# tuffy/libdvd-audio

Hardware: AMD Instinct MI355X
Metric: decoded PCM Msamples/s (bit-exact) on 6ch/96k/24b MLP (higher is better)
Workload: dtype int32 (int64 accumulate)

## Files before the change

### libdvd-audio_amd/csrc/mlp_ctx.h

```cpp
#pragma once
#include <vector>

#include "hip_ws.h"
#include "mlp_decode.h"
#include "mlp_conceal.h"
#include "mlp_index.h"

using namespace mlp;

constexpr uint32_t EV_RING = 256;
constexpr uint32_t SEQ_ROUND = 1024;

struct DecodeSettings {
    uint32_t lanes_per_seg = 0;
    uint32_t pcm_layout = DVDA_PCM_PLANAR;
    uint32_t chain_form = 0;
    const int32_t *d_init_fir = nullptr;
};

struct ConcealInfo {
    uint32_t valid, status;
    uint64_t rows, frames;
};

struct ConcealState {
    bool on = false;
    dvda_mlp_hip_ctx *child = nullptr;
    DevBuf<ConcealPlan> d_plan;
    DevBuf<uint8_t> d_bytes;
    DevBuf<uint64_t> d_tab;
    DevBuf<int32_t> d_scr[CONCEAL_ROUNDS];
    DevBuf<ConcealOp> d_ops;
    DevBuf<int32_t> d_fir;
    DevBuf<int32_t> d_edge_fir;
    bool ran = false;
    std::vector<StreamRec> h_streams;
    std::vector<dvda_mlp_conceal_edges> edges;
    std::vector<std::vector<dvda_mlp_conceal_span>> spans;
    std::vector<ConcealInfo> info;

    ~ConcealState() { dvda_mlp_hip_destroy(child); }
};

struct PresentState {
    uint32_t mode = DVDA_PRESENT_FULL;
    dvda_mlp_hip_ctx *child = nullptr;
    DevBuf<uint8_t> d_bytes;
    uint64_t bound = 0;
    DevBuf<uint32_t> d_info;
    DevBuf<uint32_t> d_size;
    DevBuf<uint32_t> d_sbase;
    DevBuf<uint32_t> d_len;
    DevBuf<uint32_t> d_base;
    DevBuf<uint64_t> d_off64, d_len64;
    Event ev[2];
    bool ev_set = false;
    bool map_valid = false;
    uint32_t h_nseg = 0;
    std::vector<SegRec> h_seg;
    std::vector<uint32_t> h_sbase, h_base, h_info;
    std::vector<StreamRec> h_streams;

    ~PresentState() { dvda_mlp_hip_destroy(child); }
};

struct dvda_mlp_hip_ctx {
    int device;
    uint32_t coop_min_seg;
    uint32_t max_streams, max_segments;
    DevBuf<uint8_t> d_masks;
    DevBuf<uint16_t> d_parts;
    DevBuf<uint32_t> d_tile_count;
    DevBuf<uint32_t> d_tile_base;
    DevBuf<uint64_t> d_cand_off;
    DevBuf<SegRec> d_seg;
    DevBuf<uint32_t> d_seg_frames;
    DevBuf<uint32_t> d_seg_fbase;
    DevBuf<uint32_t> d_seg_status;
    DevBuf<uint32_t> d_seg_rows;
    DevBuf<StreamRec> d_streams;
    uint32_t *d_n_cand;
    DevBuf<uint32_t> d_scan_tmp;
    DevBuf<int32_t> d_iir;
    DevBuf<uint32_t> d_mat;
    DevBuf<unsigned long long> d_dbg;
    DevBuf<int32_t> d_fir;
    DevBuf<uint32_t> d_seg_meta;
    DevBuf<uint32_t> d_yield;
    DevBuf<uint32_t> d_seg_check;
    DevBuf<uint32_t> d_cls;
    DevBuf<uint32_t> d_shape_key;
    DevBuf<uint64_t> d_soff, d_slen;
    DevBuf<uint32_t> d_rank;
    DevBuf<uint32_t> d_sorted_cnt;
    DevBuf<uint32_t> d_sorted_base;
    DevBuf<uint32_t> d_lane_seg;
    DevBuf<DecodeSummary> d_summary;
    DecodeSummary *h_summary;
    Stream st_aux;
    Event ev_fork, ev_join;
    DevBuf<uint32_t> d_seq_list;
    DevBuf<uint4> d_plan;
    DevBuf<uint4> d_scan4_tmp;
    DevBuf<uint32_t> d_def_list;
    DevBuf<uint32_t> d_head_list;
    DevBuf<uint32_t> d_chain_order;
    DevBuf<uint32_t> d_chain_hist;
    DevBuf<int32_t> d_fb;
    uint32_t rsv_segs;
    DevBuf<int32_t> d_res;
    DevBuf<uint32_t> d_brec;
    DevBuf<uint32_t> d_frec;
    uint32_t iir_lanes;
    DevBuf<dvda_pcm_crc_desc> d_rep_desc;
    DevBuf<uint64_t> d_rep_out;
    DevBuf<uint32_t> d_rep_work;
    DecodeSettings set;
    const uint8_t *d_bytes;
    uint64_t total_bytes;
    const uint64_t *d_stream_off;
    const uint64_t *d_stream_len;
    uint32_t n_streams;
    uint64_t tiles;
    bool indexed;
    bool small_input;
    bool decoded;
    GraphExec idx_graph;
    const void *idx_key[4];
    uint64_t idx_key_bytes;
    uint32_t idx_key_streams;
    int idx_graph_state;
    Event ev[2 * EV_RING];
    Event ev_end[EV_RING];
    uint64_t ev_count;
    ConcealState cc;
    PresentState pp;

    uint32_t fb_slots() const { return (uint32_t)(d_fb.cap / FB_WORDS); }
    ~dvda_mlp_hip_ctx() { (void)hipHostFree(h_summary); }
};

static WsCaps ws_caps(const dvda_mlp_hip_ctx *c)
{
    WsCaps w;
    w.res = c->d_res.cap;
    w.brec = c->d_brec.cap;
    w.frec = c->d_frec.cap;
    w.fb = c->d_fb.cap;
    w.max_seg = c->max_segments;
    w.max_streams = c->max_streams;
    w.lanes = c->iir_lanes;
    w.pad = 0;
    return w;
}

static inline dvda_mlp_hip_ctx *pp_inner(const dvda_mlp_hip_ctx *c)
{
    return c && c->pp.mode == DVDA_PRESENT_SUBSTREAM0 ? c->pp.child : nullptr;
}

// ... 24 lines not shown
```

### libdvd-audio_amd/csrc/mlp_hip.hip

```cpp
#include <hip/hip_runtime.h>
#include <math.h>
#include <stdint.h>
#include <stdio.h>
#include <stdlib.h>
#include <string.h>
#include <new>
#include <vector>

#include "../../include/dvda_mlp_hip.h"
#include "mlp_step.h"
#include "mlp_decode.h"
#include "mlp_chain.h"
#include "mlp_chain_small.h"
#include "mlp_check.h"
#include "mlp_coop.h"
#include "mlp_index.h"
#include "mlp_conceal.h"
#include "mlp_present.h"
#include "pcm_unswizzle.h"
#include "wav_pack.h"
#include "pcm_digest.h"
#include "pcm_levels.h"

#include "mlp_ctx.h"
#include "mlp_conceal_run.h"
#include "mlp_present_run.h"
#include "mlp_stepper.h"
#include "mlp_tiers.h"
#include "pcm_report_run.h"

extern "C" int dvda_mlp_hip_bounds_violations(unsigned long long *out4)
{
    if (!out4)
        return DVDA_HIP_EINVAL;
    out4[0] = out4[1] = out4[2] = out4[3] = 0;
#if defined(DVDA_BOUNDS)
    HIP_TRY(hipDeviceSynchronize());
    HIP_TRY(hipMemcpyFromSymbol(out4, HIP_SYMBOL(mlp::g_bounds), 4 * sizeof(unsigned long long)));
    return 1;
#else
    return DVDA_HIP_OK;
#endif
}

extern "C" const char *dvda_mlp_hip_version(void) { return "dvda-mlp-hip 0.1 (gfx950)"; }

extern "C" int dvda_mlp_hip_create(dvda_mlp_hip_ctx **out, int device, uint32_t max_streams,
                                   uint32_t max_segments)
{
    if (!out || max_streams == 0 || max_segments == 0)
        return DVDA_HIP_EINVAL;
    int ndev = 0;
    if (hipGetDeviceCount(&ndev) != hipSuccess || ndev <= 0 || device < 0 || device >= ndev) {
        fprintf(stderr, "dvda_mlp_hip: no usable HIP device (count=%d, requested=%d)\n", ndev, device);
        return DVDA_HIP_ENODEV;
    }
    HIP_TRY(hipSetDevice(device));
    dvda_mlp_hip_ctx *c = new (std::nothrow) dvda_mlp_hip_ctx();
    if (!c)
        return DVDA_HIP_ENOMEM;
    c->device = device;
    {
        int cus = 0;
        if (hipDeviceGetAttribute(&cus, hipDeviceAttributeMultiprocessorCount, device) != hipSuccess || cus <= 0)
            cus = 256;
        c->coop_min_seg = (uint32_t)cus * 4u * 64u * 7u / 4u;
        if (const char *e = getenv("DVDA_COOP_MIN_SEG"))
            c->coop_min_seg = (uint32_t)strtoul(e, nullptr, 10);
    }
    c->max_streams = max_streams;
    c->max_segments = max_segments;
    c->idx_graph_state = getenv("DVDA_INDEX_GRAPH") && atoi(getenv("DVDA_INDEX_GRAPH")) == 0 ? -1 : 0;
    const size_t ns = (size_t)max_segments, nt = (size_t)max_streams;
    c->iir_lanes = (uint32_t)(((2 * ns + DEC_THREADS - 1) / DEC_THREADS) * DEC_THREADS);
    const size_t nl = c->iir_lanes;
    hipError_t e = hipSuccess;
    auto alloc = [&](auto &buf, size_t n) {
        if (e == hipSuccess)
            e = buf.alloc(n);
    };
    alloc(c->d_cand_off, ns);
    alloc(c->d_seg, ns + 4);
    alloc(c->d_seg_frames, ns + 1);
    alloc(c->d_seg_fbase, ns + 5);
    alloc(c->d_seg_status, ns + 4);
    alloc(c->d_seg_rows, ns);
    alloc(c->d_streams, nt);
    alloc(c->d_iir, nl * MAXCH * 16);
    alloc(c->d_mat, nl * MAXMAT * 5);
    alloc(c->d_dbg, 32);
    alloc(c->d_fir, nl * 6 * 8);
    alloc(c->d_seg_meta, nl + 4);
    alloc(c->d_yield, ns);
    alloc(c->d_seg_check, 2 * ns);
    alloc(c->d_cls, 4);
    alloc(c->d_shape_key, nt);
    alloc(c->d_soff, nt);
    alloc(c->d_slen, nt);
    alloc(c->d_rank, nt);
    alloc(c->d_sorted_cnt, nt + 1);
    alloc(c->d_sorted_base, nt + 1);
    alloc(c->d_lane_seg, ns);
    alloc(c->d_summary, 1 + SUMMARY_PARTS);
    alloc(c->d_seq_list, nt);
    alloc(c->d_plan, ns + 5);
    alloc(c->d_scan4_tmp, ns / 1024 + 4);
    alloc(c->d_def_list, ns);
    alloc(c->d_head_list, ns);
    alloc(c->d_chain_order, ns);
    alloc(c->d_chain_hist, 2 * CHAIN_BUCKETS);
    if (e == hipSuccess)
        e = hipHostMalloc((void **)&c->h_summary, sizeof(DecodeSummary), hipHostMallocDefault);
    if (e == hipSuccess)
        e = hipStreamCreateWithFlags(c->st_aux.put(), hipStreamNonBlocking);
    if (e == hipSuccess)
        e = hipEventCreateWithFlags(c->ev_fork.put(), hipEventDisableTiming);
    if (e == hipSuccess)
        e = hipEventCreateWithFlags(c->ev_join.put(), hipEventDisableTiming);
    if (e == hipSuccess)
        e = hipMemset(c->d_dbg, 0, 32 * sizeof(unsigned long long));
    if (e == hipSuccess)
        e = hipMemset(c->d_seg_meta, 0, nl * sizeof(uint32_t));
    for (uint32_t i = 0; e == hipSuccess && i < 2 * EV_RING; i++)
        e = hipEventCreate(c->ev[i].put());
    for (uint32_t i = 0; e == hipSuccess && i < EV_RING; i++)
        e = hipEventCreate(c->ev_end[i].put());
    if (e != hipSuccess) {
        fprintf(stderr, "dvda_mlp_hip: workspace allocation failed: %s\n", hipGetErrorString(e));
        delete c;
        return DVDA_HIP_ENOMEM;
    }
    *out = c;
    return DVDA_HIP_OK;
}

extern "C" void dvda_mlp_hip_destroy(dvda_mlp_hip_ctx *c)
{
    if (!c)
        return;
    (void)hipSetDevice(c->device);
#if defined(DVDA_BOUNDS)
    if (getenv("DVDA_BOUNDS_REPORT")) {
        unsigned long long v[4] = {0, 0, 0, 0};
        (void)dvda_mlp_hip_bounds_violations(v);
        fprintf(stderr, "dvda_mlp_hip: bounds violations: %llu", v[0]);
        if (v[0])
            fprintf(stderr, " (first: tag %llu index %llu capacity %llu)", v[1], v[2], v[3]);
        fprintf(stderr, "\n");
    }
#endif
    delete c;
}

static int ensure_byte_ws(dvda_mlp_hip_ctx *c, uint64_t total_bytes)
{
    const uint64_t chunks = (total_bytes + 15) / 16 + 4;
    const uint64_t tiles = (chunks + IDX_TILE_CHUNKS - 1) / IDX_TILE_CHUNKS;
    auto grow_pair = [](auto &a, uint64_t na, auto &b, uint64_t nb) {
        if (na <= a.cap)
            return DVDA_HIP_OK;
        a.release();
        b.release();
        if (a.alloc(na) == hipSuccess && b.alloc(nb) == hipSuccess)
            return DVDA_HIP_OK;
        a.release();
        return DVDA_HIP_ENOMEM;
    };
    int rc = grow_pair(c->d_masks, chunks, c->d_parts, chunks + 72);
    if (rc)
        return rc;
    uint64_t most = tiles > c->max_segments ? tiles : c->max_segments;
    if (c->max_streams > most)
        most = c->max_streams;
    if ((rc = c->d_scan_tmp.grow_exact((most + 1023) / 1024 + 2)) != 0)
        return rc;
    return grow_pair(c->d_tile_count, tiles + 1, c->d_tile_base, tiles + 1);
}

__global__ void k_init_streams(StreamRec *s, uint32_t n, uint32_t *seg_status, uint32_t *seg_rows, uint32_t *yield_req,
                               uint32_t *seg_meta, uint32_t n_seg, uint32_t *cls, uint32_t *summary_words)
{
    const uint32_t i = blockIdx.x * blockDim.x + threadIdx.x;
    if (i < 4)
        cls[i] = 0;
    if (i < (1 + SUMMARY_PARTS) * sizeof(DecodeSummary) / sizeof(uint32_t))
        summary_words[i] = 0;
    if (i < n_seg) {
        seg_status[i] = 0;
        seg_rows[i] = 0;
        yield_req[i] = 0;
        seg_meta[2 * (size_t)i] = seg_meta[2 * (size_t)i + 1] = 0;
    }
    if (i < n) {
        StreamRec r;
        r.first_seg = 0xFFFFFFFFu;
        r.n_seg = 0;
        r.sync = 0;
        r.status = 0;
        r.frames = 0;
        r.consumed = 0;
        r.rows = 0;
        s[i] = r;
    }
}

__global__ void k_reset_segments(uint32_t *seg_status, uint32_t *seg_rows, uint32_t *yield_req, uint32_t *seg_meta,
                                 uint32_t n_seg)
{
    const uint32_t i = blockIdx.x * blockDim.x + threadIdx.x;
    if (i < n_seg) {
        seg_status[i] = 0;
        seg_rows[i] = 0;
        yield_req[i] = 0;
        seg_meta[2 * (size_t)i] = seg_meta[2 * (size_t)i + 1] = 0;
    }
}

__device__ __forceinline__ void check_ranges_block(const uint64_t *__restrict__ off, const uint64_t *__restrict__ len,
                                                   uint32_t n, uint64_t total_bytes, uint64_t *__restrict__ soff,
                                                   uint64_t *__restrict__ slen, StreamRec *__restrict__ streams,
                                                   unsigned long long *s_max)
{
    const uint32_t per = (n + 1023u) / 1024u;
    const uint32_t lo = threadIdx.x * per, hi = lo + per < n ? lo + per : n;
    auto end_of = [&](uint32_t i) {
        const uint64_t o = off[i], l = len[i];
        return (o <= total_bytes && l <= total_bytes - o && (o & 15u) == 0) ? o + l : 0;
    };
    unsigned long long m = 0;
    for (uint32_t i = lo; i < hi; i++) {
        const unsigned long long e = end_of(i);
        m = e > m ? e : m;
    }
    s_max[threadIdx.x] = m;
    __syncthreads();
    for (uint32_t d = 1; d < 1024u; d <<= 1) {
        const unsigned long long v = threadIdx.x >= d ? s_max[threadIdx.x - d] : 0ull;
        __syncthreads();
        if (v > s_max[threadIdx.x])
            s_max[threadIdx.x] = v;
        __syncthreads();
    }
    unsigned long long run = threadIdx.x ? s_max[threadIdx.x - 1] : 0ull;
    for (uint32_t i = lo; i < hi; i++) {
        const uint64_t o = off[i], l = len[i];
        const bool ok = (o & 15u) == 0 && o <= total_bytes && l <= total_bytes - o && o >= run;
        const uint64_t so = ok ? o : run;
        soff[i] = so < total_bytes ? so : total_bytes;
        slen[i] = ok ? l : 0;
        if (!ok)
            streams[i].status = ST_ENVELOPE | (1u << 16);
        const unsigned long long e = end_of(i);
        run = e > run ? e : run;
    }
}

__global__ __launch_bounds__(1024) void k_check_ranges(const uint64_t *__restrict__ off, const uint64_t *__restrict__ len,
                                                       uint32_t n, uint64_t total_bytes, uint64_t *__restrict__ soff,
                                                       uint64_t *__restrict__ slen, StreamRec *__restrict__ streams)
{
    __shared__ unsigned long long s_max[1024];
    check_ranges_block(off, len, n, total_bytes, soff, slen, streams, s_max);
}

constexpr uint64_t SMALL_INPUT_BYTES = 4096u * 1024u;

static void enqueue_index(dvda_mlp_hip_ctx *c, hipStream_t st, const uint8_t *d_bytes, uint64_t total_bytes,
                          const uint64_t *d_stream_off, const uint64_t *d_stream_len, uint32_t n_streams)
{
    const uint64_t tiles = c->tiles;
    const uint32_t ms = c->max_segments;
    {
        uint32_t n_init = n_streams > ms ? n_streams : ms;
        if (n_init < 1024)
            n_init = 1024;
        hipLaunchKernelGGL(k_init_streams, dim3((n_init + 255) / 256), dim3(256), 0, st, c->d_streams,
                           n_streams, c->d_seg_status, c->d_seg_rows, c->d_yield, c->d_seg_meta, ms, c->d_cls,
                           reinterpret_cast<uint32_t *>(c->d_summary.p));
        hipLaunchKernelGGL(k_check_ranges, dim3(1), dim3(1024), 0, st, d_stream_off, d_stream_len, n_streams, total_bytes,
                           c->d_soff, c->d_slen, c->d_streams);
        d_stream_off = c->d_soff;
        d_stream_len = c->d_slen;
    }
    hipLaunchKernelGGL(k_sync_mask, dim3((unsigned)tiles), dim3(IDX_THREADS), 0, st, d_bytes,
                       total_bytes, c->d_masks, c->d_tile_count, c->d_parts);
    enqueue_exscan(st, c->d_tile_count, c->d_tile_base, c->d_scan_tmp, (uint32_t)tiles, nullptr, (uint32_t)tiles);
    hipLaunchKernelGGL(k_sync_scatter, dim3((unsigned)tiles), dim3(IDX_THREADS), 0, st, c->d_masks,
                       total_bytes, c->d_tile_base, c->d_cand_off, ms);
    hipLaunchKernelGGL(k_chase, dim3((ms + 255) / 256), dim3(256), 0, st, d_bytes, d_stream_off,
                       d_stream_len, n_streams, c->d_cand_off, c->d_n_cand, ms, c->d_seg,
                       c->d_seg_frames, c->d_streams, c->d_cls);
    hipLaunchKernelGGL(k_mark_dead, dim3((ms + 255) / 256), dim3(256), 0, st, d_stream_off, d_stream_len,
                       c->d_n_cand, ms, c->d_seg, c->d_seg_frames, c->d_streams);
    enqueue_exscan(st, c->d_seg_frames, c->d_seg_fbase, c->d_scan_tmp, 0u, c->d_n_cand, ms);
    const bool pack = !(total_bytes <= SMALL_INPUT_BYTES);
    hipLaunchKernelGGL(k_link, dim3((ms + 255) / 256), dim3(256), 0, st, d_stream_off, d_stream_len,
                       c->d_n_cand, ms, c->d_seg, c->d_seg_fbase, c->d_streams, n_streams, c->d_shape_key,
                       c->d_cls + (pack ? 2 : 3));
    hipStream_t sp = st;
    bool forked = false;
    if (pack && st != nullptr && c->st_aux && hipEventRecord(c->ev_fork, st) == hipSuccess &&
        hipStreamWaitEvent(c->st_aux, c->ev_fork, 0) == hipSuccess) {
        sp = c->st_aux;
        forked = true;
    }
    if (pack) {
    hipLaunchKernelGGL(k_stream_rank, dim3((n_streams + 255) / 256), dim3(256), 0, sp, c->d_shape_key, c->d_streams,
                       n_streams, c->d_rank, c->d_sorted_cnt, c->d_cls + 2);
    enqueue_exscan(sp, c->d_sorted_cnt, c->d_sorted_base, c->d_scan_tmp, n_streams, nullptr, n_streams);
    (void)hipMemsetAsync(c->d_lane_seg, 0xFF, (size_t)ms * sizeof(uint32_t), sp);
    hipLaunchKernelGGL(k_lane_perm, dim3((ms + 255) / 256), dim3(256), 0, sp, c->d_seg, c->d_streams, c->d_n_cand, ms,
                       c->d_rank, c->d_sorted_base, c->d_cls + 2, c->d_lane_seg);
    }
    hipLaunchKernelGGL(k_au_check, dim3((unsigned)(((uint64_t)ms * CHK_GROUP + CHK_THREADS - 1) / CHK_THREADS)),
                       dim3(CHK_THREADS), 0, st, d_bytes, c->d_parts, c->d_seg, c->d_n_cand, ms, c->d_streams, c->d_seg_check);
    if (forked) {
        (void)hipEventRecord(c->ev_join, sp);
        (void)hipStreamWaitEvent(st, c->ev_join, 0);
    }
}

static int index_source(dvda_mlp_hip_ctx *c, const uint8_t *d_bytes, uint64_t total_bytes,
                        const uint64_t *d_stream_off, const uint64_t *d_stream_len, uint32_t n_streams, void *stream_)
{
    if (!c || !d_bytes || !d_stream_off || !d_stream_len || n_streams == 0 || total_bytes == 0)
        return DVDA_HIP_EINVAL;
    if (n_streams > c->max_streams)
        return DVDA_HIP_ECAPACITY;
    if (((uintptr_t)d_bytes & 15) != 0)
        return DVDA_HIP_EINVAL;
    hipStream_t st = (hipStream_t)stream_;
    HIP_TRY(hipSetDevice(c->device));
    c->cc.spans.clear();
    c->cc.info.clear();
    int rc = ensure_byte_ws(c, total_bytes);
    if (rc)
        return rc;
    c->d_bytes = d_bytes;
    c->total_bytes = total_bytes;
    c->d_stream_off = d_stream_off;
    c->d_stream_len = d_stream_len;
    c->n_streams = n_streams;
    const uint64_t chunks = (total_bytes + 15) / 16;
    const uint64_t tiles = (chunks + IDX_TILE_CHUNKS - 1) / IDX_TILE_CHUNKS;
    c->tiles = tiles;
    c->d_n_cand = c->d_tile_base + tiles;

    c->small_input = total_bytes <= SMALL_INPUT_BYTES;
    const bool same = c->idx_graph_state > 0 && c->idx_key[0] == d_bytes && c->idx_key[1] == d_stream_off &&
                      c->idx_key[2] == d_stream_len && c->idx_key[3] == (const void *)st &&
                      c->idx_key_bytes == total_bytes && c->idx_key_streams == n_streams;
    if (c->idx_graph_state == 2 && same) {
        if (hipGraphLaunch(c->idx_graph, st) == hipSuccess) {
            c->indexed = true;
            c->decoded = false;
            return DVDA_HIP_OK;
        }
        (void)hipGetLastError();
        c->idx_graph_state = -1;
    } else if (c->idx_graph_state == 1 && same && st != nullptr) {
        hipGraph_t g = nullptr;
        bool ok = hipStreamBeginCapture(st, hipStreamCaptureModeThreadLocal) == hipSuccess;
        if (ok) {
            enqueue_index(c, st, d_bytes, total_bytes, d_stream_off, d_stream_len, n_streams);
            ok = hipStreamEndCapture(st, &g) == hipSuccess && g != nullptr;
        }
        if (ok) {
            ok = hipGraphInstantiate(c->idx_graph.put(), g, nullptr, nullptr, 0) == hipSuccess;
        }
        if (g)
            (void)hipGraphDestroy(g);
        if (ok && hipGraphLaunch(c->idx_graph, st) == hipSuccess) {
            c->idx_graph_state = 2;
            c->indexed = true;
            c->decoded = false;
            return DVDA_HIP_OK;
        }
        (void)hipGetLastError();
        c->idx_graph_state = -1;
    } else if (c->idx_graph_state >= 0) {
        c->idx_key[0] = d_bytes;
// ... 608 lines not shown
```

### libdvd-audio_amd/csrc/mlp_index.h

```cpp
#pragma once
#include <hip/hip_runtime.h>
#include <stdint.h>
#include "mlp_tables.h"

namespace mlp {

struct SegRec {
    uint64_t off;
    uint64_t end;
    uint32_t stream;
    uint32_t nframes;
    uint32_t flags;
    uint32_t sync;
    uint32_t ndrop;
    uint32_t prev;
};
constexpr uint32_t SYNC_PARAMS = 0x00FFFFFFu;
constexpr uint32_t MAX_DROP = 64;

struct StreamRec {
    uint32_t first_seg;
    uint32_t n_seg;
    uint32_t sync;
    uint32_t status;
    uint64_t frames;
    uint64_t consumed;
    uint64_t rows;
};

constexpr int IDX_THREADS = 256;
constexpr int IDX_CHUNKS_PER_THREAD = 16;
constexpr int IDX_TILE_CHUNKS = IDX_THREADS * IDX_CHUNKS_PER_THREAD;

__device__ __forceinline__ uint32_t ld_u8(const uint8_t *p, uint64_t i) { return p[i]; }

__device__ __forceinline__ bool sync_frame_at(const uint8_t *b, uint64_t p, uint64_t limit)
{
    if (p + 32 > limit)
        return false;
    const uint32_t size = 2u * (((ld_u8(b, p) & 0x0Fu) << 8) | ld_u8(b, p + 1));
    if (size < 32)
        return false;
    if (ld_u8(b, p + 4) != 0xF8 || ld_u8(b, p + 5) != 0x72 || ld_u8(b, p + 6) != 0x6F ||
        ld_u8(b, p + 7) != 0xBB)
        return false;
    const uint32_t count = ld_u8(b, p + 20) >> 4;
    return count == 1 || count == 2;
}

__device__ __forceinline__ uint64_t ld_hdr8(const uint8_t *b, uint64_t p)
{
    const uint16_t *h = reinterpret_cast<const uint16_t *>(b + p);
    return (uint64_t)h[0] | ((uint64_t)h[1] << 16) | ((uint64_t)h[2] << 32) | ((uint64_t)h[3] << 48);
}

__device__ __forceinline__ bool sync_frame_hdr(const uint8_t *b, uint64_t p, uint64_t limit, uint64_t hdr)
{
    if (p + 32 > limit)
        return false;
    const uint32_t size = 2u * ((((uint32_t)hdr & 0x0Fu) << 8) | (((uint32_t)hdr >> 8) & 0xFFu));
    if (size < 32 || (uint32_t)(hdr >> 32) != 0xBB6F72F8u)
        return false;
    const uint32_t count = ld_u8(b, p + 20) >> 4;
    return count == 1 || count == 2;
}

__device__ __forceinline__ uint32_t packed_sync_at(const uint8_t *b, uint64_t p)
{
    return (ld_u8(b, p + 8) >> 4) | ((ld_u8(b, p + 8) & 0xFu) << 4) | ((ld_u8(b, p + 9) >> 4) << 8) |
           ((ld_u8(b, p + 9) & 0xFu) << 12) | ((ld_u8(b, p + 11) & 0x1Fu) << 16) | ((ld_u8(b, p + 20) >> 4) << 24);
}

__device__ const CheckTables d_chk = make_check();

__device__ __forceinline__ uint32_t mask_chunk(const uint8_t *__restrict__ bytes, uint64_t total_bytes, uint64_t chunk,
                                               const uint8_t *s_slice, uint32_t &part)
{
    const uint4 *q = reinterpret_cast<const uint4 *>(bytes) + chunk;
    const uint4 a = q[0], c = q[1];
    uint32_t w[8] = {a.x, a.y, a.z, a.w, c.x, c.y, c.z, c.w};
    uint32_t m = 0;
    uint32_t any = 0;
#pragma unroll
    for (int k = 1; k <= 4; k++) {
        const uint32_t y = w[k] ^ 0x72F872F8u;
        any |= (y - 0x00010001u) & ~y & 0x80008000u;
    }
    if (__builtin_expect(any != 0, 0)) {
#pragma unroll
        for (int j = 0; j < 8; j++) {
            const int h = j + 2;
            const uint32_t lo = (h & 1) ? (w[h >> 1] >> 16) : (w[h >> 1] & 0xFFFFu);
            const uint32_t hi = ((h + 1) & 1) ? (w[(h + 1) >> 1] >> 16) : (w[(h + 1) >> 1] & 0xFFFFu);
            if (lo == 0x72F8u && hi == 0xBB6Fu) {
                if (sync_frame_at(bytes, chunk * 16 + 2 * j, total_bytes))
                    m |= 1u << j;
            }
        }
    }
    uint32_t c0 = 0;
#pragma unroll
    for (int k = 0; k < 4; k++)
        c0 ^= s_slice[(15 - 4 * k) * 256 + (w[k] & 0xFFu)] ^ s_slice[(14 - 4 * k) * 256 + ((w[k] >> 8) & 0xFFu)] ^
              s_slice[(13 - 4 * k) * 256 + ((w[k] >> 16) & 0xFFu)] ^ s_slice[(12 - 4 * k) * 256 + (w[k] >> 24)];
    uint32_t px = w[0] ^ w[1] ^ w[2] ^ w[3];
    px ^= px >> 16;
    px = (px ^ (px >> 8)) & 0xFFu;
    part = c0 | (px << 8);
    return m;
}

__global__ __launch_bounds__(IDX_THREADS) void k_sync_mask(const uint8_t *__restrict__ bytes,
                                                           uint64_t total_bytes,
                                                           uint8_t *__restrict__ masks,
                                                           uint32_t *__restrict__ tile_count,
// ... 23 lines not shown
        s_cnt[threadIdx.x >> 6] = cnt;
    __syncthreads();
    if (threadIdx.x == 0) {
        uint32_t t = 0;
        for (int i = 0; i < IDX_THREADS / 64; i++)
            t += s_cnt[i];
        tile_count[blockIdx.x] = t;
    }
}

__global__ __launch_bounds__(1024) void k_exscan_u32(const uint32_t *__restrict__ in,
                                                     uint32_t *__restrict__ out, uint32_t n_host,
                                                     const uint32_t *__restrict__ n_ptr,
                                                     uint32_t n_cap)
{
    __shared__ uint32_t s_part[1024];
    uint32_t n = n_ptr ? *n_ptr : n_host;
    if (n > n_cap)
        n = n_cap;
    const uint32_t per = (n + 1023) / 1024;
    const uint32_t lo = threadIdx.x * per;
    const uint32_t hi = lo + per < n ? lo + per : n;
    uint32_t sum = 0;
    for (uint32_t i = lo; i < hi; i++)
        sum += in[i];
    s_part[threadIdx.x] = sum;
    __syncthreads();
    for (int o = 1; o < 1024; o <<= 1) {
        uint32_t v = threadIdx.x >= (uint32_t)o ? s_part[threadIdx.x - o] : 0;
        __syncthreads();
        s_part[threadIdx.x] += v;
        __syncthreads();
    }
    uint32_t run = threadIdx.x ? s_part[threadIdx.x - 1] : 0;
    for (uint32_t i = lo; i < hi; i++) {
        const uint32_t v = in[i];
        out[i] = run;
        run += v;
    }
    if (threadIdx.x == 1023)
        out[n] = s_part[1023];
}

__global__ __launch_bounds__(1024) void k_scan_blocks(const uint32_t *__restrict__ in,
                                                      uint32_t *__restrict__ out,
                                                      uint32_t *__restrict__ block_sum, uint32_t n_host,
                                                      const uint32_t *__restrict__ n_ptr, uint32_t n_cap)
{
    __shared__ uint32_t s_v[1024];
    uint32_t n = n_ptr ? *n_ptr : n_host;
    if (n > n_cap)
        n = n_cap;
    const uint32_t i = blockIdx.x * 1024 + threadIdx.x;
    const uint32_t v = i < n ? in[i] : 0;
    s_v[threadIdx.x] = v;
    __syncthreads();
    for (int o = 1; o < 1024; o <<= 1) {
        const uint32_t t = threadIdx.x >= (uint32_t)o ? s_v[threadIdx.x - o] : 0;
        __syncthreads();
        s_v[threadIdx.x] += t;
        __syncthreads();
    }
    if (i < n)
        out[i] = s_v[threadIdx.x] - v;
    if (threadIdx.x == 1023)
        block_sum[blockIdx.x] = s_v[1023];
}

__global__ __launch_bounds__(1024) void k_scan_add(uint32_t *__restrict__ out,
                                                   const uint32_t *__restrict__ block_base,
                                                   uint32_t n_blocks, uint32_t n_host,
                                                   const uint32_t *__restrict__ n_ptr, uint32_t n_cap)
{
    uint32_t n = n_ptr ? *n_ptr : n_host;
    if (n > n_cap)
        n = n_cap;
    const uint32_t i = blockIdx.x * 1024 + threadIdx.x;
    if (i < n)
        out[i] += block_base[blockIdx.x];
    if (i == 0)
        out[n] = block_base[n_blocks];
}

__global__ __launch_bounds__(IDX_THREADS) void k_sync_scatter(const uint8_t *__restrict__ masks,
                                                              uint64_t total_bytes,
                                                              const uint32_t *__restrict__ tile_base,
                                                              uint64_t *__restrict__ cand_off,
                                                              uint32_t max_cand)
{
    __shared__ uint32_t s_wave[IDX_THREADS / 64];
    const uint64_t n_chunks = (total_bytes + 15) >> 4;
    const uint64_t first = (uint64_t)blockIdx.x * IDX_TILE_CHUNKS +
                           (uint64_t)threadIdx.x * IDX_CHUNKS_PER_THREAD;
    static_assert(IDX_CHUNKS_PER_THREAD == 16, "one 16-byte load of mask bytes per thread");
    uint8_t m[IDX_CHUNKS_PER_THREAD];
    uint32_t cnt = 0;
    if (first + IDX_CHUNKS_PER_THREAD <= n_chunks) {
        const uint4 q = *reinterpret_cast<const uint4 *>(masks + first);
        const uint32_t w[4] = {q.x, q.y, q.z, q.w};
#pragma unroll
        for (int k = 0; k < IDX_CHUNKS_PER_THREAD; k++)
            m[k] = (uint8_t)(w[k >> 2] >> (8 * (k & 3)));
        cnt = __popc(q.x) + __popc(q.y) + __popc(q.z) + __popc(q.w);
    } else {
#pragma unroll
        for (int k = 0; k < IDX_CHUNKS_PER_THREAD; k++) {
            m[k] = (first + k < n_chunks) ? masks[first + k] : 0;
            cnt += __popc((uint32_t)m[k]);
        }
    }
    uint32_t inc = cnt;
#pragma unroll
    for (int o = 1; o < 64; o <<= 1) {
        const uint32_t v = __shfl_up(inc, o, 64);
        if ((int)(threadIdx.x & 63) >= o)
            inc += v;
    }
    if ((threadIdx.x & 63) == 63)
        s_wave[threadIdx.x >> 6] = inc;
    __syncthreads();
    uint32_t before = 0;
    for (uint32_t w = 0; w < (threadIdx.x >> 6); w++)
        before += s_wave[w];
    uint32_t at = tile_base[blockIdx.x] + before + inc - cnt;
    if (cnt == 0)
        return;
#pragma unroll
    for (int k = 0; k < IDX_CHUNKS_PER_THREAD; k++) {
        uint32_t mk = m[k];
        while (mk) {
            const int j = __ffs(mk) - 1;
            mk &= mk - 1;
            if (at < max_cand)
                cand_off[at] = (first + k) * 16 + 2 * j;
            at++;
        }
    }
}

__device__ __forceinline__ uint32_t find_stream(const uint64_t *__restrict__ stream_off,
                                                uint32_t n_streams, uint64_t p)
{
    uint32_t lo = 0, hi = n_streams;
    while (hi - lo > 1) {
        const uint32_t mid = (lo + hi) >> 1;
        if (stream_off[mid] <= p)
            lo = mid;
        else
            hi = mid;
    }
    return lo;
}

constexpr uint32_t SEG_DEAD = 1u << 24;

__device__ __forceinline__ void chase_one(uint32_t i, const uint8_t *__restrict__ bytes,
                                          const uint64_t *__restrict__ stream_off,
                                          const uint64_t *__restrict__ stream_len, uint32_t n_streams,
                                          const uint64_t *__restrict__ cand_off, SegRec *__restrict__ seg,
                                          uint32_t *__restrict__ seg_frames, StreamRec *__restrict__ streams,
                                          uint32_t *__restrict__ cls)
{
    const uint64_t off = cand_off[i];
    const uint32_t s = find_stream(stream_off, n_streams, off);
    const uint64_t s_begin = stream_off[s];
    const uint64_t s_end = s_begin + stream_len[s];
    SegRec r;
    r.off = off;
    r.stream = s;
    r.flags = 0;
    r.nframes = 0;
    r.sync = 0;
    r.ndrop = 0;
    r.prev = 0xFFFFFFFFu;
    uint64_t p = off;
    const bool outside = off >= s_end;
    if (outside) {
        r.flags = SEG_DEAD;
        r.end = off;
    } else if ((off - s_begin) & 1) {
        r.flags = 1u << 16;
        r.end = off;
    } else if (!sync_frame_at(bytes, off, s_end)) {
        r.flags = SEG_DEAD;
        r.end = off;
    } else {
        r.sync = packed_sync_at(bytes, off);
        const bool own = sync_frame_at(bytes, s_begin, s_end) &&
                         ((packed_sync_at(bytes, s_begin) ^ r.sync) & SYNC_PARAMS) == 0;
        uint32_t n = 0;
        uint64_t hdr = ld_hdr8(bytes, p);
        for (;;) {
            if (p + 4 > s_end) {
                if (p != s_end)
                    r.flags |= 1u << 21;
                break;
            }
            const uint32_t size = 2u * ((((uint32_t)hdr & 0x0Fu) << 8) | (((uint32_t)hdr >> 8) & 0xFFu));
            if (size < 4) {
                r.flags |= 1u << 4;
                break;
            }
            if (p + size > s_end) {
                r.flags |= 1u << 21;
                break;
            }
            p += size;
// ... 25 lines not shown
}

__global__ __launch_bounds__(256) void k_chase(const uint8_t *__restrict__ bytes,
                                               const uint64_t *__restrict__ stream_off,
                                               const uint64_t *__restrict__ stream_len,
                                               uint32_t n_streams,
                                               const uint64_t *__restrict__ cand_off,
                                               const uint32_t *__restrict__ n_cand_ptr,
                                               uint32_t max_cand, SegRec *__restrict__ seg,
                                               uint32_t *__restrict__ seg_frames,
                                               StreamRec *__restrict__ streams, uint32_t *__restrict__ cls)
{
    const uint32_t i = blockIdx.x * blockDim.x + threadIdx.x;
    uint32_t n_cand = *n_cand_ptr;
    if (n_cand > max_cand)
        n_cand = max_cand;
    if (i >= n_cand)
        return;
    chase_one(i, bytes, stream_off, stream_len, n_streams, cand_off, seg, seg_frames, streams, cls);
}


constexpr uint32_t STEP_CAP = 4096;
__device__ __forceinline__ void mark_dead_one(uint32_t i, uint32_t n_cand, const uint64_t *__restrict__ stream_off,
                                              const uint64_t *__restrict__ stream_len, SegRec *__restrict__ seg,
                                              uint32_t *__restrict__ seg_frames, const StreamRec *__restrict__ streams)
{
    if (i >= n_cand || i == 0)
        return;
    const uint32_t s = seg[i].stream;
    const uint64_t off = seg[i].off;
    if (seg[i - 1].stream != s)
        return;
    const uint32_t want = streams[s].sync & SYNC_PARAMS;
    const bool foreign = (seg[i].sync & SYNC_PARAMS) != want;
    uint32_t steps = 0;
    if (!foreign) {
        uint32_t seen = 0;
        for (uint32_t q = i; q-- > 0 && seen <= MAX_DROP + 1 && seg[q].stream == s;) {
            if (++steps > STEP_CAP) {
                seg[i].flags |= 1u << 16;
                return;
            }
            if ((seg[q].sync & SYNC_PARAMS) != want)
                continue;
            seen++;
            if (seg[q].end == off)
                return;
        }
    }
    const uint64_t s_end = stream_off[s] + stream_len[s];
    uint32_t seen_b = 0;
    for (uint32_t q = i; q-- > 0 && seen_b <= MAX_DROP + 1 && seg[q].stream == s;) {
        const uint64_t e = seg[q].end;
        if (++steps > STEP_CAP) {
            seg[i].flags |= 1u << 16;
            return;
        }
        if ((seg[q].sync & SYNC_PARAMS) != want)
            continue;
        seen_b++;
        if (e <= off || seg[q].nframes == 0)
            continue;
        bool lands = (e == s_end) || (seg[q].flags & (1u << 21));
        uint32_t seen_f = 0;
        for (uint32_t j = i + 1; !lands && j < n_cand && seen_f <= MAX_DROP + 1 && seg[j].stream == s && seg[j].off <= e; j++) {
            lands = seg[j].off == e;
            if ((seg[j].sync & SYNC_PARAMS) == want)
                seen_f++;
        }
        if (lands) {
            seg[i].flags |= SEG_DEAD;
            seg[i].nframes = 0;
            seg_frames[i] = 0;
            return;
        }
    }
}

__global__ __launch_bounds__(256) void k_mark_dead(const uint64_t *__restrict__ stream_off,
                                                   const uint64_t *__restrict__ stream_len,
                                                   const uint32_t *__restrict__ n_cand_ptr, uint32_t max_cand,
                                                   SegRec *__restrict__ seg, uint32_t *__restrict__ seg_frames,
                                                   const StreamRec *__restrict__ streams)
{
    const uint32_t i = blockIdx.x * blockDim.x + threadIdx.x;
    uint32_t n_cand = *n_cand_ptr;
    if (n_cand > max_cand)
        n_cand = max_cand;
    mark_dead_one(i, n_cand, stream_off, stream_len, seg, seg_frames, streams);
}

__device__ __forceinline__ uint32_t stream_shape_key(const SegRec &r)
{
    const uint32_t rows = (r.nframes - r.ndrop) * rows_per_au((r.sync >> 8) & 0xFu);
    return ((rows > 0xFFFFu ? 0xFFFFu : rows) << 16) | (((r.sync >> 8) & 0xFu) << 8) | ((r.sync >> 16) & 0x1Fu);
}

__device__ __forceinline__ void link_one(uint32_t i, uint32_t n_cand, bool overflow,
                                         const uint64_t *__restrict__ stream_off,
                                         const uint64_t *__restrict__ stream_len, SegRec *__restrict__ seg,
                                         const uint32_t *__restrict__ seg_fbase, StreamRec *__restrict__ streams,
                                         uint32_t n_streams, uint32_t *__restrict__ shape_key, uint32_t *__restrict__ hetero)
{
    if (i >= n_cand)
        return;
    if (overflow && i == n_cand - 1) {
        for (uint32_t t = seg[i].stream; t < n_streams; t++)
            atomicOr(&streams[t].status, 1u << 22);
    }
    SegRec r = seg[i];
    if (r.flags & SEG_DEAD)
        return;
    const uint32_t s = r.stream;
    const uint64_t s_begin = stream_off[s];
    const uint64_t s_end = s_begin + stream_len[s];
    uint32_t j = i + 1;
    while (j < n_cand && seg[j].stream == s && (seg[j].flags & SEG_DEAD))
        j++;
    const bool last = (j == n_cand) || (seg[j].stream != s);
    {
        uint32_t p = i;
        uint32_t prev = 0xFFFFFFFFu;
        while (p > streams[s].first_seg) {
            p--;
            if (!(seg[p].flags & SEG_DEAD)) {
                prev = p;
                break;
            }
        }
        seg[i].prev = prev;
    }
    uint32_t st = r.flags;
    if (streams[s].first_seg == i) {
        shape_key[s] = stream_shape_key(r);
        uint32_t t = 0;
        while (t < n_streams && streams[t].first_seg == 0xFFFFFFFFu)
            t++;
        if (t < n_streams && stream_shape_key(seg[streams[t].first_seg]) != shape_key[s])
            *hetero = 1u;
    }
    if (streams[s].first_seg == i && r.off != s_begin)
        st |= 1u << 0;
    if (!last && seg[j].off != r.end)
        st |= 1u << 16;
    if (r.ndrop)
        st |= 1u << 1;
    if ((r.sync ^ streams[s].sync) & SYNC_PARAMS) {
        st |= (1u << 1) | (1u << 16);
    }
    if (st != r.flags) {
        r.flags = st;
        seg[i].flags = st;
    }
    if (st)
        atomicOr(&streams[s].status, st);
    if (last) {
        streams[s].n_seg = j - streams[s].first_seg;
        streams[s].consumed = r.end - s_begin;
        streams[s].frames = seg_fbase[j] - seg_fbase[streams[s].first_seg];
        (void)s_end;
    }
}

__global__ __launch_bounds__(256) void k_link(const uint64_t *__restrict__ stream_off,
                                              const uint64_t *__restrict__ stream_len,
                                              const uint32_t *__restrict__ n_cand_ptr,
                                              uint32_t max_cand, SegRec *__restrict__ seg,
                                              const uint32_t *__restrict__ seg_fbase,
                                              StreamRec *__restrict__ streams, uint32_t n_streams,
                                              uint32_t *__restrict__ shape_key, uint32_t *__restrict__ hetero)
{
    const uint32_t i = blockIdx.x * blockDim.x + threadIdx.x;
    uint32_t n_cand = *n_cand_ptr;
    const bool overflow = n_cand > max_cand;
    if (n_cand > max_cand)
        n_cand = max_cand;
    link_one(i, n_cand, overflow, stream_off, stream_len, seg, seg_fbase, streams, n_streams, shape_key, hetero);
}

__global__ __launch_bounds__(256) void k_stream_rank(const uint32_t *__restrict__ shape_key,
                                                     const StreamRec *__restrict__ streams, uint32_t n_streams,
                                                     uint32_t *__restrict__ rank, uint32_t *__restrict__ sorted_cnt,
                                                     const uint32_t *__restrict__ hetero)
{
    __shared__ __attribute__((aligned(16))) uint32_t s_key[1024];
    if (*hetero == 0)
        return;
    const uint32_t s = blockIdx.x * blockDim.x + threadIdx.x;
    const bool live = s < n_streams;
    const uint32_t mine = live && streams[s].first_seg != 0xFFFFFFFFu ? shape_key[s] : 0u;
    const uint32_t blk_lo = blockIdx.x * blockDim.x, blk_hi = blk_lo + blockDim.x;
    uint32_t before = 0;
    for (uint32_t t0 = 0; t0 < n_streams; t0 += 1024) {
        __syncthreads();
        for (uint32_t i = threadIdx.x; i < 1024; i += blockDim.x) {
            const uint32_t t = t0 + i;
            s_key[i] = t < n_streams && streams[t].first_seg != 0xFFFFFFFFu ? shape_key[t] : 0u;
        }
        __syncthreads();
        const uint32_t lim = n_streams - t0 < 1024u ? n_streams - t0 : 1024u;
        if (t0 + 1024u <= blk_lo || t0 >= blk_hi) {
            const uint32_t bump = t0 + 1024u <= blk_lo ? 1u : 0u;
            const uint4 *k4 = reinterpret_cast<const uint4 *>(s_key);
            uint32_t i = 0;
            for (; i + 4 <= lim; i += 4) {
                const uint4 k = k4[i >> 2];
                before += (k.x + bump > mine ? 1u : 0u) + (k.y + bump > mine ? 1u : 0u) + (k.z + bump > mine ? 1u : 0u) +
                          (k.w + bump > mine ? 1u : 0u);
            }
            for (; i < lim; i++)
                before += s_key[i] + bump > mine ? 1u : 0u;
        } else {
            for (uint32_t i = 0; i < lim; i++) {
                const uint32_t k = s_key[i];
                before += (k > mine || (k == mine && t0 + i < s)) ? 1u : 0u;
            }
        }
    }
    if (!live)
        return;
    rank[s] = before;
    sorted_cnt[before] = streams[s].first_seg != 0xFFFFFFFFu ? streams[s].n_seg : 0u;
}

__global__ __launch_bounds__(256) void k_lane_perm(const SegRec *__restrict__ seg, const StreamRec *__restrict__ streams,
                                                   const uint32_t *__restrict__ n_cand_ptr, uint32_t max_cand,
                                                   const uint32_t *__restrict__ rank, const uint32_t *__restrict__ sorted_base,
                                                   const uint32_t *__restrict__ hetero, uint32_t *__restrict__ lane_seg)
{
    if (*hetero == 0)
        return;
    const uint32_t i = blockIdx.x * blockDim.x + threadIdx.x;
    uint32_t n_cand = *n_cand_ptr;
    if (n_cand > max_cand)
        n_cand = max_cand;
    if (i >= n_cand)
        return;
    const uint32_t s = seg[i].stream;
    const uint32_t first = streams[s].first_seg;
    if (first == 0xFFFFFFFFu || i < first || i - first >= streams[s].n_seg)
        return;
    lane_seg[sorted_base[rank[s]] + (i - first)] = i;
}

}
```

Baseline: 266,700.

## Fuse range check, tile scan and frame scan into index kernels

Moves the stream range check into an extra block of k_sync_scatter. Each scatter block now computes its own tile base from the preceding tile counts when the input is small, so the separate exscan launch is skipped. The segment-frame exclusive scan is replaced by per-group sums written in k_mark_dead plus a decoupled prefix computed inside k_link, which also derives per-stream frame totals. This cuts several small kernel launches and serial scan passes from the indexing phase, at the cost of redundant reads of group sums in every block and more complex cross-group stream handling.

```diff
diff --git a/libdvd-audio_amd/csrc/mlp_ctx.h b/libdvd-audio_amd/csrc/mlp_ctx.h
--- a/libdvd-audio_amd/csrc/mlp_ctx.h
+++ b/libdvd-audio_amd/csrc/mlp_ctx.h
@@ -76,6 +76,7 @@
     DevBuf<SegRec> d_seg;
     DevBuf<uint32_t> d_seg_frames;
     DevBuf<uint32_t> d_seg_fbase;
+    DevBuf<uint32_t> d_seg_gsum;
     DevBuf<uint32_t> d_seg_status;
     DevBuf<uint32_t> d_seg_rows;
     DevBuf<StreamRec> d_streams;
diff --git a/libdvd-audio_amd/csrc/mlp_hip.hip b/libdvd-audio_amd/csrc/mlp_hip.hip
--- a/libdvd-audio_amd/csrc/mlp_hip.hip
+++ b/libdvd-audio_amd/csrc/mlp_hip.hip
@@ -83,6 +83,7 @@
     alloc(c->d_seg, ns + 4);
     alloc(c->d_seg_frames, ns + 1);
     alloc(c->d_seg_fbase, ns + 5);
+    alloc(c->d_seg_gsum, ns / IDX_GROUP + 1);
     alloc(c->d_seg_status, ns + 4);
     alloc(c->d_seg_rows, ns);
     alloc(c->d_streams, nt);
@@ -216,53 +217,6 @@
     }
 }
 
-__device__ __forceinline__ void check_ranges_block(const uint64_t *__restrict__ off, const uint64_t *__restrict__ len,
-                                                   uint32_t n, uint64_t total_bytes, uint64_t *__restrict__ soff,
-                                                   uint64_t *__restrict__ slen, StreamRec *__restrict__ streams,
-                                                   unsigned long long *s_max)
-{
-    const uint32_t per = (n + 1023u) / 1024u;
-    const uint32_t lo = threadIdx.x * per, hi = lo + per < n ? lo + per : n;
-    auto end_of = [&](uint32_t i) {
-        const uint64_t o = off[i], l = len[i];
-        return (o <= total_bytes && l <= total_bytes - o && (o & 15u) == 0) ? o + l : 0;
-    };
-    unsigned long long m = 0;
-    for (uint32_t i = lo; i < hi; i++) {
-        const unsigned long long e = end_of(i);
-        m = e > m ? e : m;
-    }
-    s_max[threadIdx.x] = m;
-    __syncthreads();
-    for (uint32_t d = 1; d < 1024u; d <<= 1) {
-        const unsigned long long v = threadIdx.x >= d ? s_max[threadIdx.x - d] : 0ull;
-        __syncthreads();
-        if (v > s_max[threadIdx.x])
-            s_max[threadIdx.x] = v;
-        __syncthreads();
-    }
-    unsigned long long run = threadIdx.x ? s_max[threadIdx.x - 1] : 0ull;
-    for (uint32_t i = lo; i < hi; i++) {
-        const uint64_t o = off[i], l = len[i];
-        const bool ok = (o & 15u) == 0 && o <= total_bytes && l <= total_bytes - o && o >= run;
-        const uint64_t so = ok ? o : run;
-        soff[i] = so < total_bytes ? so : total_bytes;
-        slen[i] = ok ? l : 0;
-        if (!ok)
-            streams[i].status = ST_ENVELOPE | (1u << 16);
-        const unsigned long long e = end_of(i);
-        run = e > run ? e : run;
-    }
-}
-
-__global__ __launch_bounds__(1024) void k_check_ranges(const uint64_t *__restrict__ off, const uint64_t *__restrict__ len,
-                                                       uint32_t n, uint64_t total_bytes, uint64_t *__restrict__ soff,
-                                                       uint64_t *__restrict__ slen, StreamRec *__restrict__ streams)
-{
-    __shared__ unsigned long long s_max[1024];
-    check_ranges_block(off, len, n, total_bytes, soff, slen, streams, s_max);
-}
-
 constexpr uint64_t SMALL_INPUT_BYTES = 4096u * 1024u;
 
 static void enqueue_index(dvda_mlp_hip_ctx *c, hipStream_t st, const uint8_t *d_bytes, uint64_t total_bytes,
@@ -270,6 +224,7 @@
 {
     const uint64_t tiles = c->tiles;
     const uint32_t ms = c->max_segments;
+    const bool pack = !(total_bytes <= SMALL_INPUT_BYTES);
     {
         uint32_t n_init = n_streams > ms ? n_streams : ms;
         if (n_init < 1024)
@@ -277,26 +232,25 @@
         hipLaunchKernelGGL(k_init_streams, dim3((n_init + 255) / 256), dim3(256), 0, st, c->d_streams,
                            n_streams, c->d_seg_status, c->d_seg_rows, c->d_yield, c->d_seg_meta, ms, c->d_cls,
                            reinterpret_cast<uint32_t *>(c->d_summary.p));
-        hipLaunchKernelGGL(k_check_ranges, dim3(1), dim3(1024), 0, st, d_stream_off, d_stream_len, n_streams, total_bytes,
-                           c->d_soff, c->d_slen, c->d_streams);
-        d_stream_off = c->d_soff;
-        d_stream_len = c->d_slen;
-    }
+    }
+    const RangeCheck rc = {d_stream_off, d_stream_len, c->d_soff, c->d_slen, c->d_streams, n_streams};
+    d_stream_off = c->d_soff;
+    d_stream_len = c->d_slen;
+    static_assert(SMALL_INPUT_BYTES / (IDX_TILE_CHUNKS * 16) <= IDX_GROUP, "a small input's tiles are one group");
     hipLaunchKernelGGL(k_sync_mask, dim3((unsigned)tiles), dim3(IDX_THREADS), 0, st, d_bytes,
                        total_bytes, c->d_masks, c->d_tile_count, c->d_parts);
-    enqueue_exscan(st, c->d_tile_count, c->d_tile_base, c->d_scan_tmp, (uint32_t)tiles, nullptr, (uint32_t)tiles);
-    hipLaunchKernelGGL(k_sync_scatter, dim3((unsigned)tiles), dim3(IDX_THREADS), 0, st, c->d_masks,
-                       total_bytes, c->d_tile_base, c->d_cand_off, ms);
+    if (pack)
+        enqueue_exscan(st, c->d_tile_count, c->d_tile_base, c->d_scan_tmp, (uint32_t)tiles, nullptr, (uint32_t)tiles);
+    hipLaunchKernelGGL(k_sync_scatter, dim3((unsigned)tiles + 1u), dim3(IDX_THREADS), 0, st, c->d_masks,
+                       total_bytes, c->d_tile_count, c->d_tile_base, (uint32_t)tiles, !pack, c->d_cand_off, ms, rc);
     hipLaunchKernelGGL(k_chase, dim3((ms + 255) / 256), dim3(256), 0, st, d_bytes, d_stream_off,
                        d_stream_len, n_streams, c->d_cand_off, c->d_n_cand, ms, c->d_seg,
                        c->d_seg_frames, c->d_streams, c->d_cls);
     hipLaunchKernelGGL(k_mark_dead, dim3((ms + 255) / 256), dim3(256), 0, st, d_stream_off, d_stream_len,
-                       c->d_n_cand, ms, c->d_seg, c->d_seg_frames, c->d_streams);
-    enqueue_exscan(st, c->d_seg_frames, c->d_seg_fbase, c->d_scan_tmp, 0u, c->d_n_cand, ms);
-    const bool pack = !(total_bytes <= SMALL_INPUT_BYTES);
+                       c->d_n_cand, ms, c->d_seg, c->d_seg_frames, c->d_streams, c->d_seg_gsum);
     hipLaunchKernelGGL(k_link, dim3((ms + 255) / 256), dim3(256), 0, st, d_stream_off, d_stream_len,
-                       c->d_n_cand, ms, c->d_seg, c->d_seg_fbase, c->d_streams, n_streams, c->d_shape_key,
-                       c->d_cls + (pack ? 2 : 3));
+                       c->d_n_cand, ms, c->d_seg, c->d_seg_frames, c->d_seg_gsum, c->d_seg_fbase, c->d_streams, n_streams,
+                       c->d_shape_key, c->d_cls + (pack ? 2 : 3));
     hipStream_t sp = st;
     bool forked = false;
     if (pack && st != nullptr && c->st_aux && hipEventRecord(c->ev_fork, st) == hipSuccess &&
diff --git a/libdvd-audio_amd/csrc/mlp_index.h b/libdvd-audio_amd/csrc/mlp_index.h
--- a/libdvd-audio_amd/csrc/mlp_index.h
+++ b/libdvd-audio_amd/csrc/mlp_index.h
@@ -31,6 +31,23 @@
 constexpr int IDX_THREADS = 256;
 constexpr int IDX_CHUNKS_PER_THREAD = 16;
 constexpr int IDX_TILE_CHUNKS = IDX_THREADS * IDX_CHUNKS_PER_THREAD;
+constexpr uint32_t IDX_GROUP = 256;
+
+__device__ __forceinline__ uint32_t block_sum(uint32_t v, uint32_t *s4)
+{
+#pragma unroll
+    for (int o = 32; o > 0; o >>= 1)
+        v += __shfl_xor(v, o, 64);
+    __syncthreads();
+    if ((threadIdx.x & 63) == 0)
+        s4[threadIdx.x >> 6] = v;
+    __syncthreads();
+    uint32_t t = 0;
+#pragma unroll
+    for (int i = 0; i < IDX_THREADS / 64; i++)
+        t += s4[i];
+    return t;
+}
 
 __device__ __forceinline__ uint32_t ld_u8(const uint8_t *p, uint64_t i) { return p[i]; }
 
@@ -220,15 +237,79 @@
         out[n] = block_base[n_blocks];
 }
 
+template <uint32_t NT>
+__device__ __forceinline__ void check_ranges_block(const uint64_t *__restrict__ off, const uint64_t *__restrict__ len,
+                                                   uint32_t n, uint64_t total_bytes, uint64_t *__restrict__ soff,
+                                                   uint64_t *__restrict__ slen, StreamRec *__restrict__ streams,
+                                                   unsigned long long *s_max)
+{
+    const uint32_t per = (n + NT - 1u) / NT;
+    const uint32_t lo = threadIdx.x * per, hi = lo + per < n ? lo + per : n;
+    auto end_of = [&](uint32_t i) {
+        const uint64_t o = off[i], l = len[i];
+        return (o <= total_bytes && l <= total_bytes - o && (o & 15u) == 0) ? o + l : 0;
+    };
+    unsigned long long m = 0;
+    for (uint32_t i = lo; i < hi; i++) {
+        const unsigned long long e = end_of(i);
+        m = e > m ? e : m;
+    }
+    s_max[threadIdx.x] = m;
+    __syncthreads();
+    for (uint32_t d = 1; d < NT; d <<= 1) {
+        const unsigned long long v = threadIdx.x >= d ? s_max[threadIdx.x - d] : 0ull;
+        __syncthreads();
+        if (v > s_max[threadIdx.x])
+            s_max[threadIdx.x] = v;
+        __syncthreads();
+    }
+    unsigned long long run = threadIdx.x ? s_max[threadIdx.x - 1] : 0ull;
+    for (uint32_t i = lo; i < hi; i++) {
+        const uint64_t o = off[i], l = len[i];
+        const bool ok = (o & 15u) == 0 && o <= total_bytes && l <= total_bytes - o && o >= run;
+        const uint64_t so = ok ? o : run;
+        soff[i] = so < total_bytes ? so : total_bytes;
+        slen[i] = ok ? l : 0;
+        if (!ok)
+            streams[i].status = (1u << 9) | (1u << 16);
+        const unsigned long long e = end_of(i);
+        run = e > run ? e : run;
+    }
+}
+
+struct RangeCheck {
+    const uint64_t *off, *len;
+    uint64_t *soff, *slen;
+    StreamRec *streams;
+    uint32_t n;
+};
+
 __global__ __launch_bounds__(IDX_THREADS) void k_sync_scatter(const uint8_t *__restrict__ masks,
                                                               uint64_t total_bytes,
-                                                              const uint32_t *__restrict__ tile_base,
+                                                              const uint32_t *__restrict__ tile_count,
+                                                              uint32_t *__restrict__ tile_base, uint32_t tiles,
+                                                              bool own_base,
                                                               uint64_t *__restrict__ cand_off,
-                                                              uint32_t max_cand)
+                                                              uint32_t max_cand, RangeCheck rc)
 {
     __shared__ uint32_t s_wave[IDX_THREADS / 64];
+    __shared__ uint32_t s_sum[IDX_THREADS / 64];
+    __shared__ unsigned long long s_max[IDX_THREADS];
+    if (rc.n && blockIdx.x == 0) {
+        check_ranges_block<IDX_THREADS>(rc.off, rc.len, rc.n, total_bytes, rc.soff, rc.slen, rc.streams, s_max);
+        return;
+    }
+    const uint32_t tile = blockIdx.x - (rc.n ? 1u : 0u);
+    static_assert(IDX_GROUP <= IDX_THREADS, "a lane per tile in front");
+    uint32_t front = 0;
+    if (own_base) {
+        if (threadIdx.x < tile)
+            front = tile_count[threadIdx.x];
+    } else if (threadIdx.x == 0) {
+        front = tile_base[tile];
+    }
     const uint64_t n_chunks = (total_bytes + 15) >> 4;
-    const uint64_t first = (uint64_t)blockIdx.x * IDX_TILE_CHUNKS +
+    const uint64_t first = (uint64_t)tile * IDX_TILE_CHUNKS +
                            (uint64_t)threadIdx.x * IDX_CHUNKS_PER_THREAD;
     static_assert(IDX_CHUNKS_PER_THREAD == 16, "one 16-byte load of mask bytes per thread");
     uint8_t m[IDX_CHUNKS_PER_THREAD];
@@ -254,13 +335,28 @@
         if ((int)(threadIdx.x & 63) >= o)
             inc += v;
     }
-    if ((threadIdx.x & 63) == 63)
+#pragma unroll
+    for (int o = 32; o > 0; o >>= 1)
+        front += __shfl_xor(front, o, 64);
+    if ((threadIdx.x & 63) == 63) {
         s_wave[threadIdx.x >> 6] = inc;
-    __syncthreads();
-    uint32_t before = 0;
+        s_sum[threadIdx.x >> 6] = front;
+    }
+    __syncthreads();
+    uint32_t before = 0, base = 0, mine = 0;
     for (uint32_t w = 0; w < (threadIdx.x >> 6); w++)
         before += s_wave[w];
-    uint32_t at = tile_base[blockIdx.x] + before + inc - cnt;
+#pragma unroll
+    for (uint32_t w = 0; w < IDX_THREADS / 64; w++) {
+        base += s_sum[w];
+        mine += s_wave[w];
+    }
+    if (threadIdx.x == 0 && own_base) {
+        tile_base[tile] = base;
+        if (tile == tiles - 1)
+            tile_base[tiles] = base + mine;
+    }
+    uint32_t at = base + before + inc - cnt;
     if (cnt == 0)
         return;
 #pragma unroll
@@ -452,13 +548,19 @@
                                                    const uint64_t *__restrict__ stream_len,
                                                    const uint32_t *__restrict__ n_cand_ptr, uint32_t max_cand,
                                                    SegRec *__restrict__ seg, uint32_t *__restrict__ seg_frames,
-                                                   const StreamRec *__restrict__ streams)
-{
+                                                   const StreamRec *__restrict__ streams,
+                                                   uint32_t *__restrict__ seg_gsum)
+{
+    __shared__ uint32_t s_sum[IDX_THREADS / 64];
+    static_assert(IDX_THREADS == IDX_GROUP, "a workgroup of the segment kernels holds one group");
     const uint32_t i = blockIdx.x * blockDim.x + threadIdx.x;
     uint32_t n_cand = *n_cand_ptr;
     if (n_cand > max_cand)
         n_cand = max_cand;
     mark_dead_one(i, n_cand, stream_off, stream_len, seg, seg_frames, streams);
+    const uint32_t t = block_sum(i < n_cand ? seg_frames[i] : 0u, s_sum);
+    if (threadIdx.x == 0)
+        seg_gsum[blockIdx.x] = t;
 }
 
 __device__ __forceinline__ uint32_t stream_shape_key(const SegRec &r)
@@ -470,8 +572,9 @@
 __device__ __forceinline__ void link_one(uint32_t i, uint32_t n_cand, bool overflow,
                                          const uint64_t *__restrict__ stream_off,
                                          const uint64_t *__restrict__ stream_len, SegRec *__restrict__ seg,
-                                         const uint32_t *__restrict__ seg_fbase, StreamRec *__restrict__ streams,
-                                         uint32_t n_streams, uint32_t *__restrict__ shape_key, uint32_t *__restrict__ hetero)
+                                         StreamRec *__restrict__ streams, uint32_t n_streams,
+                                         uint32_t *__restrict__ shape_key, uint32_t *__restrict__ hetero,
+                                         uint32_t &last_first, uint32_t &last_end)
 {
     if (i >= n_cand)
         return;
@@ -528,25 +631,111 @@
     if (last) {
         streams[s].n_seg = j - streams[s].first_seg;
         streams[s].consumed = r.end - s_begin;
-        streams[s].frames = seg_fbase[j] - seg_fbase[streams[s].first_seg];
+        last_first = streams[s].first_seg;
+        last_end = j;
         (void)s_end;
     }
+}
+
+__device__ __forceinline__ uint32_t range_part(const uint32_t *__restrict__ seg_frames,
+                                               const uint32_t *__restrict__ seg_gsum, uint32_t a, uint32_t b)
+{
+    uint32_t acc = 0;
+    const uint32_t ga = (a + IDX_GROUP - 1) / IDX_GROUP, gb = b / IDX_GROUP;
+    if (ga >= gb) {
+        for (uint32_t x = a + threadIdx.x; x < b; x += IDX_THREADS)
+            acc += seg_frames[x];
+        return acc;
+    }
+    for (uint32_t x = a + threadIdx.x; x < ga * IDX_GROUP; x += IDX_THREADS)
+        acc += seg_frames[x];
+    for (uint32_t g = ga + threadIdx.x; g < gb; g += IDX_THREADS)
+        acc += seg_gsum[g];
+    for (uint32_t x = gb * IDX_GROUP + threadIdx.x; x < b; x += IDX_THREADS)
+        acc += seg_frames[x];
+    return acc;
 }
 
 __global__ __launch_bounds__(256) void k_link(const uint64_t *__restrict__ stream_off,
                                               const uint64_t *__restrict__ stream_len,
                                               const uint32_t *__restrict__ n_cand_ptr,
                                               uint32_t max_cand, SegRec *__restrict__ seg,
-                                              const uint32_t *__restrict__ seg_fbase,
+                                              const uint32_t *__restrict__ seg_frames,
+                                              const uint32_t *__restrict__ seg_gsum,
+                                              uint32_t *__restrict__ seg_fbase,
                                               StreamRec *__restrict__ streams, uint32_t n_streams,
                                               uint32_t *__restrict__ shape_key, uint32_t *__restrict__ hetero)
 {
-    const uint32_t i = blockIdx.x * blockDim.x + threadIdx.x;
+    __shared__ uint32_t s_sum[IDX_THREADS / 64];
+    __shared__ uint32_t s_wave[IDX_THREADS / 64];
+    __shared__ uint32_t s_ex[IDX_GROUP + 1];
+    __shared__ uint32_t s_req[2][4];
+    const uint32_t lo = blockIdx.x * IDX_GROUP, hi = lo + IDX_GROUP, i = lo + threadIdx.x;
     uint32_t n_cand = *n_cand_ptr;
     const bool overflow = n_cand > max_cand;
     if (n_cand > max_cand)
         n_cand = max_cand;
-    link_one(i, n_cand, overflow, stream_off, stream_len, seg, seg_fbase, streams, n_streams, shape_key, hetero);
+    if (lo >= n_cand && lo != 0)
+        return;
+    const uint32_t v = i < n_cand ? seg_frames[i] : 0u;
+    uint32_t part = 0;
+    for (uint32_t g = threadIdx.x; g < blockIdx.x; g += IDX_THREADS)
+        part += seg_gsum[g];
+    const uint32_t gbase = block_sum(part, s_sum);
+    uint32_t inc = v;
+#pragma unroll
+    for (int o = 1; o < 64; o <<= 1) {
+        const uint32_t u = __shfl_up(inc, o, 64);
+        if ((int)(threadIdx.x & 63) >= o)
+            inc += u;
+    }
+    if ((threadIdx.x & 63) == 63)
+        s_wave[threadIdx.x >> 6] = inc;
+    if (threadIdx.x < 2)
+        s_req[threadIdx.x][1] = 0;
+    __syncthreads();
+    uint32_t ex = gbase + inc - v;
+    for (uint32_t w = 0; w < (threadIdx.x >> 6); w++)
+        ex += s_wave[w];
+    s_ex[threadIdx.x] = ex;
+    if (threadIdx.x == IDX_GROUP - 1)
+        s_ex[IDX_GROUP] = ex + v;
+    if (i < n_cand)
+        seg_fbase[i] = ex;
+    if (i + 1 == n_cand)
+        seg_fbase[n_cand] = ex + v;
+    if (n_cand == 0 && i == 0)
+        seg_fbase[0] = 0;
+    __syncthreads();
+    uint32_t first = 0xFFFFFFFFu, end = 0xFFFFFFFFu;
+    link_one(i, n_cand, overflow, stream_off, stream_len, seg, streams, n_streams, shape_key, hetero, first, end);
+    if (end != 0xFFFFFFFFu) {
+        const uint32_t a = first > lo ? first : lo, b = end < hi ? end : hi;
+        const uint32_t inner = s_ex[b - lo] - s_ex[a - lo];
+        if (first >= lo && end <= hi) {
+            streams[seg[i].stream].frames = inner;
+        } else {
+            uint32_t *q = s_req[first < lo ? 0 : 1];
+            q[0] = first;
+            q[1] = end;
+            q[2] = seg[i].stream;
+            q[3] = inner;
+        }
+    }
+    __syncthreads();
+    for (int k = 0; k < 2; k++) {
+        const uint32_t f = s_req[k][0], e = s_req[k][1];
+        if (e == 0)
+            continue;
+        uint32_t acc = 0;
+        if (f < lo)
+            acc += range_part(seg_frames, seg_gsum, f, lo);
+        if (e > hi)
+            acc += range_part(seg_frames, seg_gsum, hi, e);
+        const uint32_t out = block_sum(acc, s_sum);
+        if (threadIdx.x == 0)
+            streams[s_req[k][2]].frames = s_req[k][3] + out;
+    }
 }
 
 __global__ __launch_bounds__(256) void k_stream_rank(const uint32_t *__restrict__ shape_key,
```

New measurement: 267,500 (median of 6 runs). No clear change (+0.3%).
